# HarborC/PL-SLAM

Measured on NVIDIA H100. Metric: frames/sec (extract+match+pose-LM) 640x480, higher is better.
Workload: dtype u8/i32 front-end, f32 descriptors, f64 LM

## Files before the change

### include/plslam_b200.h

```cpp
#ifndef PLSLAM_B200_H
#define PLSLAM_B200_H
#include <stddef.h>
#include <stdint.h>
#ifdef __cplusplus
extern "C" {
#endif

#define PL_OK 0
#define PL_ERR_ARG (-1)
#define PL_ERR_CUDA (-2)
#define PL_ERR_CAPACITY (-3)

const char* pl_last_error(void);
int pl_version(void);
unsigned long long pl_launch_count(void);

typedef struct PLKeyPoint {
  float x, y, size, angle, response;
  int32_t octave, class_id;
} PLKeyPoint;

typedef struct PLOrbConfig {
  int width, height;
  int nfeatures;
// ... 61 lines not shown
                         const float* pt_inv_sigma2, const float* pt_Xw, int n_lines, const double* line_func,
                         const double* line_Xw, float* Tcw_out, uint8_t* pt_outlier, uint8_t* line_outlier,
                         int* iterations );
size_t pl_pose_optimization_scratch_doubles(int B, int cap_points, int cap_lines);
int pl_pose_optimization_dev(int mode, int B, const float* Tcw_in, const float* K, const int* n_points,
                             int cap_points, const float* pt_obs, const float* pt_inv_sigma2, const float* pt_Xw,
                             const int* n_lines, int cap_lines, const double* line_func, const double* line_Xw,
                             float* Tcw_out, uint8_t* pt_outlier, uint8_t* line_outlier, int* inliers,
                             int* iterations, double* scratch, void* stream);

typedef struct PLLineConfig {
  int width, height;
  int nfeatures;
  double min_line_length;
  int max_batch;
  int segment_cap;
  int lsd_used_in_global;
} PLLineConfig;
typedef struct PLLine PLLine;
int pl_line_create(const PLLineConfig* cfg, PLLine** out);
void pl_line_destroy(PLLine* h);
int pl_line_capacity(const PLLine* h);
int pl_line_extract(PLLine* h, const uint8_t* img, int stride, const uint8_t* mask, void* keylines, uint8_t* desc,
                    double* linefunc, int* n);
int pl_line_extract_batch(PLLine* h, const uint8_t* imgs, int stride, size_t frame_stride, int B, const uint8_t* mask,
                          void* keylines, uint8_t* desc, double* linefunc, int* n);
int pl_line_extract_batch_dev(PLLine* h, const uint8_t* imgs, int stride, size_t frame_stride, int B,
                              const uint8_t* mask, void* keylines, uint8_t* desc, double* linefunc, int* n, void* stream);
int pl_line_check_overflow(PLLine* h);
int pl_line_debug_segments(PLLine* h, int frame, float* out, int cap);
int pl_line_debug_scaled(PLLine* h, int frame, uint8_t* out, int* sw, int* sh);
int pl_line_debug_sobel(PLLine* h, int frame, short* dx, short* dy);
int pl_line_debug_order(PLLine* h, int frame, unsigned* out, int cap);
int pl_line_debug_ctl(PLLine* h, int frame, int* out, int nwords);

typedef struct PLFrontendConfig {
  int width, height, max_batch;
  int orb_nfeatures; float orb_scale_factor; int orb_nlevels, orb_ini_th, orb_min_th;
  int line_nfeatures; double line_min_length;
  int lm_cap_points, lm_cap_lines;
} PLFrontendConfig;
typedef struct PLFrontend PLFrontend;
int pl_frontend_create(const PLFrontendConfig* cfg, PLFrontend** out);
void pl_frontend_destroy(PLFrontend* h);
int pl_frontend_capacities(const PLFrontend* h, int* cap_keypoints, int* cap_lines);
int pl_frontend_set_pose_problems(PLFrontend* h, int B, const float* Tcw0, const float* K, const int* n_points,
                                  const float* pt_obs, const float* pt_inv_sigma2, const float* pt_Xw, const int* n_lines,
                                  const double* line_func, const double* line_Xw);
int pl_frontend_set_camera(PLFrontend* h, const float* K, const float* dist5);
long long pl_frontend_set_pose_problems_async(PLFrontend* h, int B, const float* Tcw0, const float* K, const int* n_points,
                                              const float* pt_obs, const float* pt_inv_sigma2, const float* pt_Xw,
                                              const int* n_lines, const double* line_func, const double* line_Xw, void* stream);
int pl_frontend_check_overflow(PLFrontend* h);
int pl_frontend_set_wrap(PLFrontend* h, int on);
int pl_frontend_set_tracking(PLFrontend* h, int on);
int pl_frontend_fetch_tracking(PLFrontend* h, int B, int which, int* point_match, int* n_point_matches, int* line_match,
                               int* n_line_matches, float* map_pos, uint8_t* point_in_view, uint8_t* line_in_view);
int pl_frontend_fetch_keys_un(PLFrontend* h, int B, PLKeyPoint* out);
int pl_frontend_run_dev(PLFrontend* h, const uint8_t* imgs, int stride, size_t frame_stride, int B, void* stream);
int pl_frontend_run(PLFrontend* h, const uint8_t* imgs, int stride, size_t frame_stride, int B, PLKeyPoint* kps,
                    uint8_t* desc, int* n, void* keylines, uint8_t* ldesc, double* linefunc, int* nl, int* pt_matches,
                    int* n_pt_matches, int* line_matches, int* n_line_matches, float* poses, int* inliers);
int pl_frontend_submit(PLFrontend* h, const uint8_t* imgs, int stride, size_t frame_stride, int B, PLKeyPoint* kps,
                       uint8_t* desc, int* n, void* keylines, uint8_t* ldesc, double* linefunc, int* nl, int* pt_matches,
                       int* n_pt_matches, int* line_matches, int* n_line_matches, float* poses, int* inliers);
int pl_frontend_wait(PLFrontend* h, int keep_in_flight);
// ... 216 lines not shown
```

### pl-slam_b200/binding.py

```python
import ctypes as C
import os
import numpy as np

_HERE = os.path.dirname(os.path.abspath(__file__))
LIB_PATH = os.environ.get("PLSLAM_B200_LIB") or os.path.join(_HERE, "libplslam_b200.so")

KP_DTYPE = np.dtype([("x", "<f4"), ("y", "<f4"), ("size", "<f4"), ("angle", "<f4"),
                     ("response", "<f4"), ("octave", "<i4"), ("class_id", "<i4")])


class PLError(RuntimeError):
    pass


class PLOrbConfig(C.Structure):
    _fields_ = [("width", C.c_int), ("height", C.c_int), ("nfeatures", C.c_int), ("scale_factor", C.c_float),
                ("nlevels", C.c_int), ("ini_th_fast", C.c_int), ("min_th_fast", C.c_int), ("max_batch", C.c_int),
                ("cell_slot_cap", C.c_int)]


_lib = None
vp = C.c_void_p


# ... 233 lines not shown


KEYLINE_DTYPE = np.dtype([("angle", "<f4"), ("class_id", "<i4"), ("octave", "<i4"), ("ptx", "<f4"), ("pty", "<f4"),
                          ("response", "<f4"), ("size", "<f4"), ("startPointX", "<f4"), ("startPointY", "<f4"),
                          ("endPointX", "<f4"), ("endPointY", "<f4"), ("sPointInOctaveX", "<f4"),
                          ("sPointInOctaveY", "<f4"), ("ePointInOctaveX", "<f4"), ("ePointInOctaveY", "<f4"),
                          ("lineLength", "<f4"), ("numOfPixels", "<i4")])


class PLLineConfig(C.Structure):
    _fields_ = [("width", C.c_int), ("height", C.c_int), ("nfeatures", C.c_int), ("min_line_length", C.c_double),
                ("max_batch", C.c_int), ("segment_cap", C.c_int), ("lsd_used_in_global", C.c_int)]


class LINEextractor:

    def __init__(self, numOctaves=1, scale=1.2, nLSDFeature=200, min_line_length=0.0, width=640, height=480, max_batch=1,
                 segment_cap=0):
        if numOctaves != 1 or int(scale) != 1:
            raise PLError("only numOctaves == 1 and int(scale) == 1 are supported (all reference configs)")
        self.cfg = PLLineConfig(width, height, nLSDFeature, float(min_line_length), max_batch, segment_cap, 0)
        self._h = vp()
        L = lib()
        L.pl_line_create.argtypes = [C.POINTER(PLLineConfig), C.POINTER(vp)]
        L.pl_line_destroy.argtypes = [vp]
        L.pl_line_capacity.argtypes = [vp]
        L.pl_line_extract.argtypes = [vp, vp, C.c_int, vp, vp, vp, vp, vp]
        L.pl_line_extract_batch.argtypes = [vp, vp, C.c_int, C.c_size_t, C.c_int, vp, vp, vp, vp, vp]
        L.pl_line_extract_batch_dev.argtypes = [vp, vp, C.c_int, C.c_size_t, C.c_int, vp, vp, vp, vp, vp, vp]
        L.pl_line_debug_segments.argtypes = [vp, C.c_int, vp, C.c_int]
        L.pl_line_debug_scaled.argtypes = [vp, C.c_int, vp, vp, vp]
        L.pl_line_debug_sobel.argtypes = [vp, C.c_int, vp, vp]
        L.pl_line_debug_order.argtypes = [vp, C.c_int, vp, C.c_int]
        check(L.pl_line_create(C.byref(self.cfg), C.byref(self._h)))
        self.capacity = check(L.pl_line_capacity(self._h))

    def __del__(self):
        if getattr(self, "_h", None) and self._h.value:
            lib().pl_line_destroy(self._h)
            self._h = vp()

    def __call__(self, image, mask=None):
        image = np.ascontiguousarray(image, np.uint8)
        if image.size == 0:
            return np.zeros(0, KEYLINE_DTYPE), np.zeros((0, 32), np.uint8), np.zeros((0, 3))
        if mask is not None and (mask.shape != image.shape or mask.dtype != np.uint8):
            raise PLError("Mask error while detecting lines: please check its dimensions and that data type is CV_8UC1")
        kl = np.zeros(self.capacity, KEYLINE_DTYPE); desc = np.zeros((self.capacity, 32), np.uint8)
        lf = np.zeros((self.capacity, 3), np.float64); n = C.c_int(0)
        m = None if mask is None else np.ascontiguousarray(mask)
        check(lib().pl_line_extract(self._h, _p(image), image.strides[0], _p(m), _p(kl), _p(desc), _p(lf), C.byref(n)))
        return kl[:n.value].copy(), desc[:n.value].copy(), lf[:n.value].copy()

    def extract_batch(self, images, mask=None):
        images = np.ascontiguousarray(images, np.uint8)
        B = images.shape[0]
        kl = np.zeros((B, self.capacity), KEYLINE_DTYPE); desc = np.zeros((B, self.capacity, 32), np.uint8)
        lf = np.zeros((B, self.capacity, 3), np.float64); n = np.zeros(B, np.int32)
        m = None if mask is None else np.ascontiguousarray(mask)
        check(lib().pl_line_extract_batch(self._h, _p(images), images.strides[1], images.strides[0], B, _p(m), _p(kl),
                                          _p(desc), _p(lf), _p(n)))
        return kl, desc, lf, n

    def extract_batch_dev(self, img_ptr, stride, frame_stride, B, mask_ptr, kl_ptr, desc_ptr, lf_ptr, n_ptr, stream=None):
        check(lib().pl_line_extract_batch_dev(self._h, img_ptr, stride, frame_stride, B, mask_ptr, kl_ptr, desc_ptr,
                                              lf_ptr, n_ptr, stream))

    def debug_segments(self, frame=0):
        n = check(lib().pl_line_debug_segments(self._h, frame, None, 0))
        out = np.zeros((max(n, 1), 4), np.float32)
        check(lib().pl_line_debug_segments(self._h, frame, _p(out), n))
        return out[:n]

    def debug_scaled(self, frame=0):
        sw, sh = C.c_int(), C.c_int()
        check(lib().pl_line_debug_scaled(self._h, frame, None, C.byref(sw), C.byref(sh)))
        out = np.zeros((sh.value, sw.value), np.uint8)
        check(lib().pl_line_debug_scaled(self._h, frame, _p(out), C.byref(sw), C.byref(sh)))
        return out

    def debug_sobel(self, frame=0):
        dx = np.zeros((self.cfg.height, self.cfg.width), np.int16); dy = np.zeros_like(dx)
        check(lib().pl_line_debug_sobel(self._h, frame, _p(dx), _p(dy)))
        return dx, dy

    def debug_order(self, frame=0):
        n = check(lib().pl_line_debug_order(self._h, frame, None, 0))
        out = np.zeros(max(n, 1), np.uint32)
        check(lib().pl_line_debug_order(self._h, frame, _p(out), n))
        return out[:n]


class PLFrontendConfig(C.Structure):
    _fields_ = [("width", C.c_int), ("height", C.c_int), ("max_batch", C.c_int), ("orb_nfeatures", C.c_int),
                ("orb_scale_factor", C.c_float), ("orb_nlevels", C.c_int), ("orb_ini_th", C.c_int), ("orb_min_th", C.c_int),
                ("line_nfeatures", C.c_int), ("line_min_length", C.c_double), ("lm_cap_points", C.c_int),
                ("lm_cap_lines", C.c_int)]


class Frontend:

    def __init__(self, width=640, height=480, max_batch=8, orb=(1000, 1.2, 8, 20, 7), lines=(200, 0.0), lm_caps=(512, 128)):
        self.cfg = PLFrontendConfig(width, height, max_batch, orb[0], orb[1], orb[2], orb[3], orb[4], lines[0], lines[1],
                                    lm_caps[0], lm_caps[1])
        self._h = vp()
        L = lib()
        L.pl_frontend_create.argtypes = [C.POINTER(PLFrontendConfig), C.POINTER(vp)]
        L.pl_frontend_destroy.argtypes = [vp]
        L.pl_frontend_capacities.argtypes = [vp, vp, vp]
        L.pl_frontend_set_pose_problems.argtypes = [vp, C.c_int] + [vp] * 9
        L.pl_frontend_run_dev.argtypes = [vp, vp, C.c_int, C.c_size_t, C.c_int, vp]
        L.pl_frontend_run.argtypes = [vp, vp, C.c_int, C.c_size_t, C.c_int] + [vp] * 13
        L.pl_frontend_io_bytes.argtypes = [vp, vp, vp]
        L.pl_frontend_fetch.argtypes = [vp, C.c_int] + [vp] * 12
        L.pl_frontend_set_timing.argtypes = [vp, C.c_int]
        L.pl_frontend_grow_ms.argtypes = [vp, vp]
        L.pl_frontend_grow_bytes_per_frame.argtypes = [vp]
        L.pl_frontend_grow_bytes_per_frame.restype = C.c_longlong
        L.pl_frontend_copy_poses_dev.argtypes = [vp, C.c_int, vp, vp]
        check(L.pl_frontend_create(C.byref(self.cfg), C.byref(self._h)))
        ck, cl = C.c_int(), C.c_int()
        check(L.pl_frontend_capacities(self._h, C.byref(ck), C.byref(cl)))
        self.capK, self.capL = ck.value, cl.value
# ... 924 lines not shown
```

### pl-slam_b200/csrc/common.cuh

```cuda
#pragma once
#include <cuda_runtime.h>
#include <stdint.h>
#include <stdio.h>
#include <string>
#include <atomic>
#include "../../include/plslam_b200.h"

namespace pl {

void set_error(const char* fmt, ...);
extern std::atomic<unsigned long long> g_launches;
inline void count_launch(int n = 1) { g_launches.fetch_add((unsigned long long)n, std::memory_order_relaxed); }

#define PL_CUDA(expr)                                                                       \
  do {                                                                                      \
    cudaError_t _e = (expr);                                                                \
    if (_e != cudaSuccess) {                                                                \
      pl::set_error("%s:%d %s -> %s", __FILE__, __LINE__, #expr, cudaGetErrorString(_e));   \
      return PL_ERR_CUDA;                                                                   \
    }                                                                                       \
  } while (0)

#define PL_LAUNCH_CHECK()                                                                   \
  do {                                                                                      \
    pl::count_launch();                                                                     \
    cudaError_t _e = cudaGetLastError();                                                    \
    if (_e != cudaSuccess) {                                                                \
      pl::set_error("%s:%d kernel launch -> %s", __FILE__, __LINE__, cudaGetErrorString(_e)); \
      return PL_ERR_CUDA;                                                                   \
    }                                                                                       \
  } while (0)

#define PL_ARG(cond)                                                                        \
  do {                                                                                      \
    if (!(cond)) {                                                                          \
      pl::set_error("%s:%d bad argument: %s", __FILE__, __LINE__, #cond);                   \
      return PL_ERR_ARG;                                                                    \
    }                                                                                       \
  } while (0)

int require_device();

template <typename T>
inline int dev_alloc(T** p, size_t n) {
  PL_CUDA(cudaMalloc((void**)p, n * sizeof(T)));
// ... 22 lines not shown
```

### pl-slam_b200/csrc/frontend.cu

```cuda

#include "common.cuh"
#include <vector>
#include <string>
#include <cstdio>
#include <string.h>

namespace pl {
__global__ void k_prev_matched_init(const PLKeyPoint* __restrict__ kps_prev, const int* __restrict__ n_prev, int cap, int B,
                                    float* __restrict__ pm) {
  const int b = blockIdx.y, i = blockIdx.x * blockDim.x + threadIdx.x;
  if (i < n_prev[b]) { pm[((long long)b * cap + i) * 2] = kps_prev[(long long)b * cap + i].x; pm[((long long)b * cap + i) * 2 + 1] = kps_prev[(long long)b * cap + i].y; }
}

__global__ void k_track_points(const PLKeyPoint* __restrict__ ku_prev, const PLKeyPoint* __restrict__ kraw_prev, const int* __restrict__ n_prev,
                               int cap, const float* __restrict__ Tcw0, const float* __restrict__ K, uint8_t* __restrict__ valid,
                               float* __restrict__ pos, int* __restrict__ oct, float* __restrict__ ang, float* __restrict__ proj,
                               float* __restrict__ vcos) {
  const int b = blockIdx.y, i = blockIdx.x * blockDim.x + threadIdx.x;
  if (i >= cap) return;
  const long long o = (long long)b * cap + i;
  const bool v = i < min(n_prev[b], cap);
  valid[o] = v ? 1 : 0;
  if (!v) return;
  const PLKeyPoint k = ku_prev[o];
// ... 103 lines not shown
  if (h->sLine) cudaStreamDestroy(h->sLine);
  if (h->sLm) cudaStreamDestroy(h->sLm);
  if (h->evStart) cudaEventDestroy(h->evStart);
  if (h->evLine) cudaEventDestroy(h->evLine);
  if (h->evLm) cudaEventDestroy(h->evLm);
  delete h;
}

extern "C" int pl_frontend_create(const PLFrontendConfig* cfg, PLFrontend** out) {
  PL_ARG(cfg && out && cfg->max_batch >= 1 && cfg->lm_cap_points >= 1 && cfg->lm_cap_lines >= 1);
  int rc = require_device();
  if (rc) return rc;
  PLFrontend* h = new PLFrontend;
  h->cfg = *cfg;
  h->B = cfg->max_batch;
#define FE_TRY(e) do { int _r = (e); if (_r) { pl_frontend_destroy(h); return _r; } } while (0)
#define FE_CUDA(e) do { cudaError_t _e = (e); if (_e != cudaSuccess) { set_error("%s -> %s", #e, cudaGetErrorString(_e)); pl_frontend_destroy(h); return PL_ERR_CUDA; } } while (0)
  PLOrbConfig oc = {cfg->width, cfg->height, cfg->orb_nfeatures, cfg->orb_scale_factor, cfg->orb_nlevels, cfg->orb_ini_th, cfg->orb_min_th, cfg->max_batch, 0};
  FE_TRY(pl_orb_create(&oc, &h->orb));
  PLLineConfig lc = {cfg->width, cfg->height, cfg->line_nfeatures, cfg->line_min_length, cfg->max_batch, 0, 0};
  FE_TRY(pl_line_create(&lc, &h->line));
  h->capK = pl_orb_capacity(h->orb); h->capL = pl_line_capacity(h->line);
  FE_CUDA(cudaStreamCreateWithFlags(&h->stream, cudaStreamNonBlocking));
  FE_CUDA(cudaStreamCreateWithFlags(&h->sLine, cudaStreamNonBlocking));
  FE_CUDA(cudaStreamCreateWithFlags(&h->sLm, cudaStreamNonBlocking));
  FE_CUDA(cudaEventCreateWithFlags(&h->evStart, cudaEventDisableTiming));
  FE_CUDA(cudaEventCreateWithFlags(&h->evLine, cudaEventDisableTiming));
  FE_CUDA(cudaEventCreateWithFlags(&h->evLm, cudaEventDisableTiming));
  { const char* e = getenv("PLSLAM_FRONTEND_OVERLAP"); h->overlap = !(e && e[0] == '0'); }
  {
    int dev = 0, sms = 132;
    FE_CUDA(cudaGetDevice(&dev));
    FE_CUDA(cudaDeviceGetAttribute(&sms, cudaDevAttrMultiProcessorCount, dev));
    h->serial_batch = 32 * sms;
  }
  if (const char* e = getenv("PLSLAM_FRONTEND_ORDER")) {
    const std::string o(e);
    if (o.size() == 3 && o.find('L') != std::string::npos && o.find('O') != std::string::npos && o.find('M') != std::string::npos) memcpy(h->order, o.data(), 3);
  }
  const size_t B = h->B, cK = h->capK, cL = h->capL, cp = cfg->lm_cap_points, cl = cfg->lm_cap_lines;
  FE_TRY(dev_alloc(&h->d_img, (size_t)cfg->width * cfg->height * B));
  FE_TRY(dev_alloc(&h->d_kps_prev, cK * (B + 1))); h->d_kps = h->d_kps_prev + cK;
  FE_TRY(dev_alloc(&h->d_desc_prev, cK * 32 * (B + 1))); h->d_desc = h->d_desc_prev + cK * 32;
  FE_TRY(dev_alloc(&h->d_n_prev, B + 1)); h->d_n = h->d_n_prev + 1;
  FE_CUDA(cudaMemset(h->d_n_prev, 0, sizeof(int) * (B + 1)));
  FE_TRY(dev_alloc(&h->d_ldesc_prev, cL * 32 * (B + 1))); h->d_ldesc = h->d_ldesc_prev + cL * 32;
  FE_TRY(dev_alloc(&h->d_nl_prev, B + 1)); h->d_nl = h->d_nl_prev + 1;
  FE_CUDA(cudaMemset(h->d_nl_prev, 0, sizeof(int) * (B + 1)));
  FE_TRY(dev_alloc(&h->d_kl_prev, cL * 68 * (B + 1))); h->d_kl = h->d_kl_prev + cL * 68;
  FE_TRY(dev_alloc(&h->d_lf, cL * 3 * B));
  FE_TRY(dev_alloc(&h->d_bounds, 4)); FE_TRY(dev_alloc(&h->d_pm, cK * 2 * B)); FE_TRY(dev_alloc(&h->d_m12, cK * B));
  FE_TRY(dev_alloc(&h->d_nm, B)); FE_TRY(dev_alloc(&h->d_scr, cK * 2 * B)); FE_TRY(dev_alloc(&h->d_lm, cL * B)); FE_TRY(dev_alloc(&h->d_nlm, B));
  float bounds[4] = {0.f, 0.f, (float)cfg->width, (float)cfg->height};
  FE_CUDA(cudaMemcpy(h->d_bounds, bounds, sizeof(bounds), cudaMemcpyHostToDevice));
  FE_TRY(dev_alloc(&h->d_T0, 16 * B)); FE_TRY(dev_alloc(&h->d_K, 4 * B)); FE_TRY(dev_alloc(&h->d_pobs, cp * 2 * B));
  FE_TRY(dev_alloc(&h->d_pw, cp * B)); FE_TRY(dev_alloc(&h->d_pX, cp * 3 * B)); FE_TRY(dev_alloc(&h->d_Tout, 16 * B * 2));
  FE_TRY(dev_alloc(&h->d_lfun, cl * 3 * B)); FE_TRY(dev_alloc(&h->d_lX, cl * 6 * B));
  FE_TRY(dev_alloc(&h->d_scratch, pl_pose_optimization_scratch_doubles((int)B, (int)cp, (int)cl)));
  FE_TRY(dev_alloc(&h->d_np, B)); FE_TRY(dev_alloc(&h->d_nl_lm, B)); FE_TRY(dev_alloc(&h->d_inl, B * 2)); FE_TRY(dev_alloc(&h->d_its, B * 2));
  FE_TRY(dev_alloc(&h->d_pout, cp * B * 2)); FE_TRY(dev_alloc(&h->d_lout, cl * B * 2));
  *out = h;
  return PL_OK;
}

extern "C" int pl_frontend_capacities(const PLFrontend* h, int* cap_keypoints, int* cap_lines) {
  PL_ARG(h);
  if (cap_keypoints) *cap_keypoints = h->capK;
// ... 434 lines not shown
```

### pl-slam_b200/csrc/line.cu

```cuda

#include "common.cuh"
#include "lsd_grow_core.cuh"
#include "libm_glibc.cuh"
#include <math.h>
#include <string.h>
#include <stdlib.h>
#include <vector>
#include <algorithm>

namespace pl {

constexpr double kPI = 3.14159265358979323846;
constexpr double kDegToRads = kPI / 180;
constexpr int kBins = 1024;
constexpr int kChunkRows = 8;


struct PLKeyLineRec {
  float angle; int class_id; int octave; float ptx, pty; float response; float size;
  float startPointX, startPointY, endPointX, endPointY;
  float sPointInOctaveX, sPointInOctaveY, ePointInOctaveX, ePointInOctaveY;
  float lineLength; int numOfPixels;
};
static_assert(sizeof(PLKeyLineRec) == 68, "KeyLine layout");

struct LineParams {
  int w, h, sw, sh, npx;
  int nchunk;
  int s_th;
  int min_reg_size;
  int seg_cap, capL, nfeatures;
  double min_line_length;
  double prec, prec_hi, p, density_th;
  float sure_ca2, sure_cn2;
};

__device__ __forceinline__ float fast_atan2_deg_l(float y, float x) {
  const float k = (float)(180.0 / 3.14159265358979323846);
  const float p1 = 0.9997878412794807f * k, p3 = -0.3258083974640975f * k;
  const float p5 = 0.1555786518463281f * k, p7 = -0.04432655554792128f * k;
  const float eps = 2.220446049250313e-16f;
  const float ax = fabsf(x), ay = fabsf(y);
  const float c = __fdiv_rn(fminf(ax, ay), __fadd_rn(fmaxf(ax, ay), eps)), c2 = __fmul_rn(c, c);
  float a = __fmul_rn(__fadd_rn(__fmul_rn(__fadd_rn(__fmul_rn(__fadd_rn(__fmul_rn(p7, c2), p5), c2), p3), c2), p1), c);
// ... 191 lines not shown
}

__global__ void __launch_bounds__(128) k_lsd_scatter(LineParams P, const int* __restrict__ S2, const int* __restrict__ maxs,
                                                     const int* __restrict__ offsets, unsigned* __restrict__ order) {
  __shared__ unsigned short cnt[4][kBins];
  const int wid = threadIdx.x >> 5, lane = threadIdx.x & 31;
  const int chunk = blockIdx.x * 4 + wid, f = blockIdx.y;
  for (int i = lane; i < kBins; i += 32) cnt[wid][i] = 0;
  __syncwarp();
  if (chunk >= P.nchunk) return;
  const int ms = maxs[f];
  const double max_grad = ms > 0 ? sqrt((double)ms / 4.0) : -1.0;
  const double bin_coef = (max_grad > 0) ? (double)(kBins - 1) / max_grad : 0.0;
  const int y0 = chunk * kChunkRows, y1 = min(y0 + kChunkRows, P.sh - 1);
  const int* SS = S2 + (long long)f * P.npx;
  const int* off = offsets + (long long)f * kBins * P.nchunk;
  unsigned* O = order + (long long)f * P.npx;
  const int n = (y1 - y0) * P.sw;
  const unsigned lt = (1u << lane) - 1u;
  for (int i0 = 0; i0 < n; i0 += 32) {
    int i = i0 + lane, bin = -1, pix = 0;
    if (i < n) {
      int y = y0 + i / P.sw, x = i % P.sw;
      pix = x | (y << 16);
      const int sv = SS[y * P.sw + x];
      if (sv > P.s_th) bin = s_bin(sv, bin_coef);
    }
    unsigned peers = __match_any_sync(0xffffffffu, bin);
    if (bin >= 0) O[off[bin * P.nchunk + chunk] + cnt[wid][bin] + __popc(peers & lt)] = (unsigned)pix;
    __syncwarp();
    if (bin >= 0 && (peers & lt) == 0) cnt[wid][bin] += (unsigned short)__popc(peers);
    __syncwarp();
  }
}

constexpr int kGrowQ = 256;
constexpr int kCommitBatches = 4;
constexpr unsigned kGrowWatchdog = 6u * 1000u * 1000u;
__device__ __forceinline__ int first_zero(unsigned m) { return m == 0xffffffffu ? 32 : __ffs(~m) - 1; }

__device__ __forceinline__ void warp_commit(const lg::Params& GP, const lg::Frame& Fm, float4* __restrict__ segs, int lane) {
  using namespace lg;
  const unsigned lt = (1u << lane) - 1u;
  for (int round = 0; round < kCommitBatches; round++) {
    const int F = ld_i(&Fm.ctl[C_FIN]);
    if (F >= Fm.n) return;
    const int i = F + lane;
    const unsigned w1 = (i < Fm.n) ? ld_u(&Fm.st[i]) : 0u;
    const unsigned s1 = w1 & ST_STATE;
    const int pre1 = first_zero(__ballot_sync(0xffffffffu, s1 == ST_NOOP || s1 == ST_EATEN || s1 == ST_DONE));
    if (pre1 == 0) return;
    __threadfence();
    unsigned w2 = 0u;
    bool ok = false;
    if (lane < pre1) { w2 = ld_u(&Fm.st[i]); ok = task_valid(GP, Fm, i, w2); }
    const int pre2 = min(pre1, first_zero(__ballot_sync(0xffffffffu, ok)));
    float4 sg;
    const bool has = (lane < pre2) && task_has_segment(Fm, w2, sg);
    const unsigned ms = __ballot_sync(0xffffffffu, has);
    const int ns = ld_i(&Fm.ctl[C_NS]);
    if (has) { const int slot = ns + __popc(ms & lt); if (slot < GP.seg_cap) segs[slot] = sg; }
    __syncwarp();
    if (lane == 0) {
      st_i(&Fm.ctl[C_NS], ns + __popc(ms));
      __threadfence();
      a_max(&Fm.ctl[C_FIN], F + pre2);
// ... 437 lines not shown
    s_norm2[0] = __fdiv_rn(1.f, sqrtf(temp));
  }
  __syncthreads();
  for (int i = tid; i < 72; i += 64) des[i] = __fmul_rn(des[i], s_norm2[0]);
  __syncthreads();
  if (tid < 32) {
    const float* f1 = &des[8 * c_comb[2 * tid]];
    const float* f2 = &des[8 * c_comb[2 * tid + 1]];
    unsigned r = 0;
#pragma unroll
    for (int i = 0; i < 8; i++) if (f1[i] > f2[i]) r += (1u << i);
    desc[((long long)f * P.capL + li) * 32 + tid] = (uint8_t)r;
  }
}

}

using namespace pl;

struct PLLine {
  PLLineConfig cfg;
  LineParams P;
  cudaStream_t stream = nullptr;
  uint8_t* d_scaled = nullptr;
  float2* d_seedcs = nullptr;
  lg::Params GP;
  int grow_warps_target = 132 * 16;
  int grow_wpf_max = 64;
  int grow_spec_max_batch = 0;
  size_t lane_warps = 0;
  int4* d_rec = nullptr; int* d_sq = nullptr;
  unsigned *d_st = nullptr, *d_pool = nullptr, *d_lanebuf = nullptr; int* d_ctl = nullptr; double* d_wtab = nullptr;
  GradRec* d_gtab = nullptr; float2* d_gtab_seed = nullptr;
  unsigned short* d_counts = nullptr;
  int *d_offsets = nullptr, *d_ndef = nullptr, *d_maxs = nullptr, *d_nseg = nullptr, *d_overflow = nullptr;
  unsigned* d_order = nullptr;
  float4* d_segs = nullptr;
  short2* d_dxy = nullptr;
  uint8_t* d_img = nullptr; PLKeyLineRec* d_kls = nullptr; uint8_t* d_desc = nullptr; double* d_lf = nullptr; int* d_nl = nullptr;
  uint8_t* d_mask = nullptr;
  size_t key_smem = 0;
  int last_B = 0;
  int timing = 0;
  cudaEvent_t ev0 = nullptr, ev1 = nullptr;
};

static const unsigned char h_comb[64] = {0, 1, 0, 2, 0, 3, 0, 4, 0, 5, 0, 6, 1, 2, 1, 3, 1, 4, 1, 5, 1, 6, 2, 3, 2, 4, 2, 5, 2, 6, 2, 7,
                                         2, 8, 3, 4, 3, 5, 3, 6, 3, 7, 3, 8, 4, 5, 4, 6, 4, 7, 4, 8, 5, 6, 5, 7, 5, 8, 6, 7, 6, 8, 7, 8};

extern "C" void pl_line_destroy(PLLine* h) {
  if (!h) return;
  cudaFree(h->d_gtab); cudaFree(h->d_gtab_seed); cudaFree(h->d_scaled); cudaFree(h->d_seedcs); cudaFree(h->d_rec); cudaFree(h->d_sq); cudaFree(h->d_st); cudaFree(h->d_pool); cudaFree(h->d_lanebuf); cudaFree(h->d_ctl); cudaFree(h->d_wtab); cudaFree(h->d_counts); cudaFree(h->d_offsets);
  cudaFree(h->d_ndef); cudaFree(h->d_maxs); cudaFree(h->d_nseg); cudaFree(h->d_overflow); cudaFree(h->d_order);
  cudaFree(h->d_segs); cudaFree(h->d_dxy); cudaFree(h->d_img); cudaFree(h->d_kls);
  cudaFree(h->d_desc); cudaFree(h->d_lf); cudaFree(h->d_nl); cudaFree(h->d_mask);
  if (h->stream) cudaStreamDestroy(h->stream);
  delete h;
}

extern "C" int pl_line_create(const PLLineConfig* cfg, PLLine** out) {
  PL_ARG(cfg && out);
  PL_ARG(cfg->width >= 64 && cfg->height >= 64 && cfg->width < 8000 && cfg->height < 8000 && cfg->nfeatures > 0 && cfg->max_batch >= 1);
  int rc = require_device();
  if (rc) return rc;
  PLLine* h = new PLLine;
  h->cfg = *cfg;
// ... 4 lines not shown
  P.nchunk = (P.sh - 1 + kChunkRows - 1) / kChunkRows;
  const double ANG_TH = 22.5, QUANT = 2.0;
  P.prec = kPI * ANG_TH / 180; P.p = ANG_TH / 180; P.density_th = 0.7;
  {
    const double twopi = 2 * kPI;
    double c = twopi - P.prec;
    while ((twopi - nextafter(c, 0.0)) <= P.prec) c = nextafter(c, 0.0);
    while (!((twopi - c) <= P.prec)) c = nextafter(c, 10.0);
    P.prec_hi = c;
  }
  {
    const double M = 0.05 * M_PI / 180.0, ca = cos(P.prec - M), cn = cos(P.prec + M);
    P.sure_ca2 = (float)(ca * ca); P.sure_cn2 = (float)(cn * cn);
  }
  const double rho = QUANT / sin(P.prec);
  int s = 0;
  while (sqrt((double)(s + 1) / 4.0) <= rho) s++;
  P.s_th = s;
  const double LOG_NT = 5 * (log10((double)P.sw) + log10((double)P.sh)) / 2 + log10(11.0);
  P.min_reg_size = (int)(size_t)(-LOG_NT / log10(P.p));
  P.seg_cap = cfg->segment_cap > 0 ? cfg->segment_cap : 8192;
  P.nfeatures = cfg->nfeatures; P.capL = cfg->nfeatures + 1; P.min_line_length = cfg->min_line_length;
  { size_t c2 = 1; while (c2 < (size_t)P.seg_cap) c2 <<= 1; h->key_smem = c2 * 8; }
  const size_t B = cfg->max_batch, npx = P.npx;
#define LN_TRY(e) do { int _r = (e); if (_r) { pl_line_destroy(h); return _r; } } while (0)
#define LN_CUDA(e) do { cudaError_t _e = (e); if (_e != cudaSuccess) { set_error("%s -> %s", #e, cudaGetErrorString(_e)); pl_line_destroy(h); return PL_ERR_CUDA; } } while (0)
  LN_CUDA(cudaStreamCreateWithFlags(&h->stream, cudaStreamNonBlocking));
  LN_TRY(dev_alloc(&h->d_scaled, npx * B)); LN_TRY(dev_alloc(&h->d_seedcs, npx * B)); LN_TRY(dev_alloc(&h->d_rec, npx * B));
  LN_TRY(dev_alloc(&h->d_sq, npx * B));
  {
    int dev = 0, sms = 132;
    cudaGetDevice(&dev); cudaDeviceGetAttribute(&sms, cudaDevAttrMultiProcessorCount, dev);
    h->grow_warps_target = sms * 16;
    if (const char* e = getenv("PLSLAM_LSD_GROW_WARPS")) { const int v = atoi(e); if (v > 0) h->grow_warps_target = v; }
    if (const char* e = getenv("PLSLAM_LSD_GROW_WPF")) { const int v = atoi(e); if (v > 0) h->grow_wpf_max = v; }
    if (const char* e = getenv("PLSLAM_LSD_GROW_SPEC_MAXB")) h->grow_spec_max_batch = atoi(e);
    lg::Params& G = h->GP;
    G.sw = P.sw; G.sh = P.sh; G.npx = P.npx; G.min_reg_size = P.min_reg_size; G.seg_cap = P.seg_cap;
    G.lane_cap = 1024; G.pool_cap = 4 * P.npx; G.window = 8192;
    if (const char* e = getenv("PLSLAM_LSD_GROW_WINDOW")) G.window = atoi(e);
    G.prec = P.prec; G.prec_hi = P.prec_hi; G.density_th = P.density_th;
    h->lane_warps = std::max<size_t>(std::min<size_t>(B * (size_t)h->grow_wpf_max, (size_t)h->grow_warps_target), B);
    LN_TRY(dev_alloc(&h->d_st, npx * B)); LN_TRY(dev_alloc(&h->d_pool, (size_t)G.pool_cap * B)); LN_TRY(dev_alloc(&h->d_ctl, (size_t)lg::kCtlStride * B));
    LN_TRY(dev_alloc(&h->d_lanebuf, h->lane_warps * 32 * (size_t)G.lane_cap));
    const int nw = 2 * kGradR * kGradR + 1;
    LN_TRY(dev_alloc(&h->d_wtab, (size_t)nw));
    k_lsd_wtab<<<(nw + 255) / 256, 256, 0, h->stream>>>(h->d_wtab, nw);
    LN_CUDA(cudaGetLastError());
    count_launch();
  }
  LN_TRY(dev_alloc(&h->d_counts, (size_t)kBins * P.nchunk * B)); LN_TRY(dev_alloc(&h->d_offsets, (size_t)kBins * P.nchunk * B));
  LN_TRY(dev_alloc(&h->d_ndef, B)); LN_TRY(dev_alloc(&h->d_maxs, B)); LN_TRY(dev_alloc(&h->d_nseg, B)); LN_TRY(dev_alloc(&h->d_overflow, 1));
  LN_TRY(dev_alloc(&h->d_order, npx * B)); LN_TRY(dev_alloc(&h->d_segs, (size_t)P.seg_cap * B));
  LN_TRY(dev_alloc(&h->d_dxy, (size_t)P.w * P.h * B));
  LN_CUDA(cudaMemset(h->d_overflow, 0, sizeof(int)));
  LN_TRY(dev_alloc(&h->d_gtab, (size_t)kGradN * kGradN)); LN_TRY(dev_alloc(&h->d_gtab_seed, (size_t)kGradN * kGradN));
  k_lsd_grad_table<<<(kGradN * kGradN + 255) / 256, 256, 0, h->stream>>>(h->d_gtab, h->d_gtab_seed);
  LN_CUDA(cudaGetLastError());
  LN_CUDA(cudaStreamSynchronize(h->stream));
  count_launch();
  {
    float gG[63], gL[21];
    double u = (7 * 3 - 1) / 2, sigma = (7 * 2 + 1) / 2, inv = -1 / (2 * sigma * sigma);
    for (int i = 0; i < 21; i++) { double d = i - u; gL[i] = (float)exp(d * d * inv); }
    u = (9 * 7 - 1) / 2; sigma = u; inv = -1 / (2 * sigma * sigma);
    for (int i = 0; i < 63; i++) { double d = i - u; gG[i] = (float)exp(d * d * inv); }
    LN_CUDA(cudaMemcpyToSymbol(c_gaussG, gG, sizeof(gG)));
    LN_CUDA(cudaMemcpyToSymbol(c_gaussL, gL, sizeof(gL)));
    LN_CUDA(cudaMemcpyToSymbol(c_comb, h_comb, sizeof(h_comb)));
  }
  LN_CUDA(cudaFuncSetAttribute(k_keylines, cudaFuncAttributeMaxDynamicSharedMemorySize, (int)h->key_smem));
  *out = h;
  return PL_OK;
}

extern "C" int pl_line_capacity(const PLLine* h) { return h ? h->P.capL : PL_ERR_ARG; }

extern "C" int pl_line_set_timing(PLLine* h, int on) {
  PL_ARG(h);
  if (on && !h->ev0) { PL_CUDA(cudaEventCreate(&h->ev0)); PL_CUDA(cudaEventCreate(&h->ev1)); }
  h->timing = on;
  return PL_OK;
}
extern "C" int pl_line_grow_ms(PLLine* h, float* ms) {
  PL_ARG(h && ms && h->ev0);
  PL_CUDA(cudaEventSynchronize(h->ev1));
  PL_CUDA(cudaEventElapsedTime(ms, h->ev0, h->ev1));
  return PL_OK;
}
extern "C" long long pl_line_grow_bytes_per_frame(const PLLine* h) { return h ? (long long)h->P.npx * 28 : 0; }

extern "C" int pl_line_extract_batch_dev(PLLine* h, const uint8_t* imgs, int stride, size_t frame_stride, int B,
                                         const uint8_t* mask, void* keylines, uint8_t* desc, double* linefunc, int* n,
                                         void* stream_) {
  PL_ARG(h && imgs && keylines && desc && linefunc && n && B >= 1 && B <= h->cfg.max_batch && stride >= h->cfg.width);
  cudaStream_t st = stream_ ? (cudaStream_t)stream_ : h->stream;
  const LineParams& P = h->P;
  h->last_B = B;
  PL_CUDA(cudaMemsetAsync(h->d_maxs, 0, sizeof(int) * B, st));
  k_lsd_scale<<<dim3((P.sw + 31) / 32, (P.sh + 31) / 32, B), 256, 0, st>>>(P, imgs, stride, (long long)frame_stride, h->d_scaled);
  PL_LAUNCH_CHECK();
  {
    const dim3 grd((P.sw + 255) / 256, (P.sh + 3) / 4, B);
    if (P.sw % 4 == 0)
      k_lsd_grad<true><<<grd, 256, 0, st>>>(P, h->d_scaled, reinterpret_cast<const float4*>(h->d_gtab), h->d_gtab_seed, h->d_rec, h->d_sq, h->d_seedcs, h->d_maxs);
    else
      k_lsd_grad<false><<<grd, 256, 0, st>>>(P, h->d_scaled, reinterpret_cast<const float4*>(h->d_gtab), h->d_gtab_seed, h->d_rec, h->d_sq, h->d_seedcs, h->d_maxs);
  }
  PL_LAUNCH_CHECK();
  k_lsd_hist<<<dim3(P.nchunk, B), 256, 0, st>>>(P, h->d_sq, h->d_maxs, h->d_counts);
  PL_LAUNCH_CHECK();
  k_lsd_scan<<<B, kBins, 0, st>>>(P, h->d_counts, h->d_offsets, h->d_ndef);
  PL_LAUNCH_CHECK();
  k_lsd_scatter<<<dim3((P.nchunk + 3) / 4, B), 128, 0, st>>>(P, h->d_sq, h->d_maxs, h->d_offsets, h->d_order);
  PL_LAUNCH_CHECK();
  if (B <= h->grow_spec_max_batch) {
    PL_CUDA(cudaMemsetAsync(h->d_st, 0, sizeof(unsigned) * (size_t)P.npx * B, st));
    k_lsd_grow_init<<<(B + 127) / 128, 128, 0, st>>>(h->d_ctl, B);
    PL_LAUNCH_CHECK();
    if (h->timing) PL_CUDA(cudaEventRecord(h->ev0, st));
    const int wpf = std::max(1, std::min(h->grow_wpf_max, h->grow_warps_target / B));
    k_lsd_grow<1><<<B * wpf, 32, 0, st>>>(P, h->GP, h->d_rec, h->d_seedcs, h->d_sq, h->d_order, h->d_ndef, h->d_st, h->d_pool, h->d_ctl,
                                          h->d_lanebuf, h->d_wtab, h->d_segs, h->d_nseg, h->d_overflow, B, wpf);
    PL_LAUNCH_CHECK();
  } else {
    if (h->timing) PL_CUDA(cudaEventRecord(h->ev0, st));
    static const int pre_maxb = getenv("PLSLAM_LSD_PRE_MAXB") ? atoi(getenv("PLSLAM_LSD_PRE_MAXB")) : 256;
    const int chunk = (int)std::min<long long>(B, 0xffffffffLL / P.npx);
    for (int b0 = 0; b0 < B; b0 += chunk) {
      const int nb = std::min(chunk, B - b0);
      const size_t po = (size_t)b0 * P.npx;
      if (B <= pre_maxb)
        k_lsd_grow_ordered<true><<<nb, 32, 0, st>>>(P, h->d_rec + po, h->d_sq + po, h->d_seedcs + po, h->d_order + po, h->d_ndef + b0,
                                                    h->d_pool + (size_t)b0 * h->GP.pool_cap, h->GP.pool_cap, h->d_st + po, h->d_wtab,
                                                    h->d_segs + (size_t)b0 * P.seg_cap, h->d_nseg + b0, h->d_overflow, nb);
      else
        k_lsd_grow_ordered<false><<<nb, 32, 0, st>>>(P, h->d_rec + po, h->d_sq + po, h->d_seedcs + po, h->d_order + po, h->d_ndef + b0,
                                                     h->d_pool + (size_t)b0 * h->GP.pool_cap, h->GP.pool_cap, h->d_st + po, h->d_wtab,
                                                     h->d_segs + (size_t)b0 * P.seg_cap, h->d_nseg + b0, h->d_overflow, nb);
    }
    PL_LAUNCH_CHECK();
  }
  if (h->timing) PL_CUDA(cudaEventRecord(h->ev1, st));
  k_keylines<<<B, 256, h->key_smem, st>>>(P, h->d_segs, h->d_nseg, mask, (PLKeyLineRec*)keylines, linefunc, n);
  PL_LAUNCH_CHECK();
  k_lbd_sobel<<<dim3((P.w + kSobOut - 1) / kSobOut, (P.h + kSobOut - 1) / kSobOut, B), 256, 0, st>>>(P, imgs, stride, (long long)frame_stride, h->d_dxy);
  PL_LAUNCH_CHECK();
  k_lbd_describe<<<dim3(P.capL, B), 64, 0, st>>>(P, (const PLKeyLineRec*)keylines, n, h->d_dxy, desc);
// ... 52 lines not shown
  return pl_line_extract_batch(h, img, stride, 0, 1, mask, keylines, desc, linefunc, n);
}

extern "C" int pl_line_debug_segments(PLLine* h, int frame, float* out, int cap) {
  PL_ARG(h && frame >= 0 && frame < h->last_B);
  int n = 0;
  PL_CUDA(cudaStreamSynchronize(h->stream));
  PL_CUDA(cudaMemcpy(&n, h->d_nseg + frame, sizeof(int), cudaMemcpyDeviceToHost));
  if (out && n) PL_CUDA(cudaMemcpy(out, h->d_segs + (size_t)frame * h->P.seg_cap, sizeof(float4) * std::min(n, cap), cudaMemcpyDeviceToHost));
  return n;
}
extern "C" int pl_line_debug_scaled(PLLine* h, int frame, uint8_t* out, int* sw, int* sh) {
  PL_ARG(h && frame >= 0 && frame < h->last_B && sw && sh);
  *sw = h->P.sw; *sh = h->P.sh;
  PL_CUDA(cudaStreamSynchronize(h->stream));
  if (out) PL_CUDA(cudaMemcpy(out, h->d_scaled + (size_t)frame * h->P.npx, h->P.npx, cudaMemcpyDeviceToHost));
  return PL_OK;
}
extern "C" int pl_line_debug_sobel(PLLine* h, int frame, short* dx, short* dy) {
  PL_ARG(h && frame >= 0 && frame < h->last_B && dx && dy);
  const size_t n = (size_t)h->P.w * h->P.h;
  PL_CUDA(cudaStreamSynchronize(h->stream));
  std::vector<short2> tmp(n);
  PL_CUDA(cudaMemcpy(tmp.data(), h->d_dxy + frame * n, n * sizeof(short2), cudaMemcpyDeviceToHost));
  for (size_t i = 0; i < n; i++) { dx[i] = tmp[i].x; dy[i] = tmp[i].y; }
  return PL_OK;
}
extern "C" int pl_line_debug_ctl(PLLine* h, int frame, int* out, int nwords) {
  PL_ARG(h && out && frame >= 0 && frame < h->cfg.max_batch && nwords > 0 && nwords <= lg::kCtlStride);
  PL_CUDA(cudaStreamSynchronize(h->stream));
  PL_CUDA(cudaMemcpy(out, h->d_ctl + (size_t)frame * lg::kCtlStride, sizeof(int) * nwords, cudaMemcpyDeviceToHost));
  return PL_OK;
}
extern "C" int pl_line_debug_order(PLLine* h, int frame, unsigned* out, int cap) {
  PL_ARG(h && frame >= 0 && frame < h->last_B);
  int n = 0;
  PL_CUDA(cudaStreamSynchronize(h->stream));
  PL_CUDA(cudaMemcpy(&n, h->d_ndef + frame, sizeof(int), cudaMemcpyDeviceToHost));
  if (out && n) {
    PL_CUDA(cudaMemcpy(out, h->d_order + (size_t)frame * h->P.npx, sizeof(unsigned) * std::min(n, cap), cudaMemcpyDeviceToHost));
    for (int i = 0; i < std::min(n, cap); i++) out[i] = (out[i] >> 16) * (unsigned)h->P.sw + (out[i] & 0xffffu);
  }
  return n;
}

#ifdef PL_GROW_STATS
extern "C" int pl_line_grow_stats(unsigned long long* out, int reset) {
  cudaDeviceSynchronize();
  if (out) cudaMemcpyFromSymbol(out, pl::ord::g_grow_stats, sizeof(unsigned long long) * 24);
  if (reset) { unsigned long long z[24] = {0}; cudaMemcpyToSymbol(pl::ord::g_grow_stats, z, sizeof(z)); }
  return 0;
}
#endif
```

Before: 10830.

## Fuse LSD seed histogram, scan and scatter into one thread-block-cluster kernel

Adds a kernel that uses an 8-CTA thread block cluster per frame to build the seed-gradient histogram, compute prefix offsets across the cluster through distributed shared memory, and scatter pixel coordinates into a shared-memory slice. The slice is then written to the global order array with vectorized stores. It replaces the three-launch hist/scan/scatter path, removing two launches and the global count and offset round trips. It is only chosen when the batch reaches 32 frames per SM, or when forced by an environment variable. The kernel needs a large dynamic shared-memory footprint, and debug entry points for the chosen path are added.

```diff
diff --git a/include/plslam_b200.h b/include/plslam_b200.h
--- a/include/plslam_b200.h
+++ b/include/plslam_b200.h
@@ -117,6 +117,8 @@
 int pl_line_debug_scaled(PLLine* h, int frame, uint8_t* out, int* sw, int* sh);
 int pl_line_debug_sobel(PLLine* h, int frame, short* dx, short* dy);
 int pl_line_debug_order(PLLine* h, int frame, unsigned* out, int cap);
+int pl_line_debug_seed_path(PLLine* h);
+int pl_line_debug_fill_order(PLLine* h, int byte);
 int pl_line_debug_ctl(PLLine* h, int frame, int* out, int nwords);
 
 typedef struct PLFrontendConfig {
diff --git a/pl-slam_b200/binding.py b/pl-slam_b200/binding.py
--- a/pl-slam_b200/binding.py
+++ b/pl-slam_b200/binding.py
@@ -289,6 +289,8 @@
         L.pl_line_debug_scaled.argtypes = [vp, C.c_int, vp, vp, vp]
         L.pl_line_debug_sobel.argtypes = [vp, C.c_int, vp, vp]
         L.pl_line_debug_order.argtypes = [vp, C.c_int, vp, C.c_int]
+        L.pl_line_debug_seed_path.argtypes = [vp]
+        L.pl_line_debug_fill_order.argtypes = [vp, C.c_int]
         check(L.pl_line_create(C.byref(self.cfg), C.byref(self._h)))
         self.capacity = check(L.pl_line_capacity(self._h))
 
@@ -346,6 +348,12 @@
         out = np.zeros(max(n, 1), np.uint32)
         check(lib().pl_line_debug_order(self._h, frame, _p(out), n))
         return out[:n]
+
+    def debug_seed_path(self):
+        return check(lib().pl_line_debug_seed_path(self._h))
+
+    def debug_fill_order(self, byte=0xFF):
+        check(lib().pl_line_debug_fill_order(self._h, byte))
 
 
 class PLFrontendConfig(C.Structure):
diff --git a/pl-slam_b200/csrc/common.cuh b/pl-slam_b200/csrc/common.cuh
--- a/pl-slam_b200/csrc/common.cuh
+++ b/pl-slam_b200/csrc/common.cuh
@@ -11,6 +11,7 @@
 void set_error(const char* fmt, ...);
 extern std::atomic<unsigned long long> g_launches;
 inline void count_launch(int n = 1) { g_launches.fetch_add((unsigned long long)n, std::memory_order_relaxed); }
+constexpr int kSerialFramesPerSM = 32;
 
 #define PL_CUDA(expr)                                                                       \
   do {                                                                                      \
diff --git a/pl-slam_b200/csrc/frontend.cu b/pl-slam_b200/csrc/frontend.cu
--- a/pl-slam_b200/csrc/frontend.cu
+++ b/pl-slam_b200/csrc/frontend.cu
@@ -159,7 +159,7 @@
     int dev = 0, sms = 132;
     FE_CUDA(cudaGetDevice(&dev));
     FE_CUDA(cudaDeviceGetAttribute(&sms, cudaDevAttrMultiProcessorCount, dev));
-    h->serial_batch = 32 * sms;
+    h->serial_batch = pl::kSerialFramesPerSM * sms;
   }
   if (const char* e = getenv("PLSLAM_FRONTEND_ORDER")) {
     const std::string o(e);
diff --git a/pl-slam_b200/csrc/line.cu b/pl-slam_b200/csrc/line.cu
--- a/pl-slam_b200/csrc/line.cu
+++ b/pl-slam_b200/csrc/line.cu
@@ -2,6 +2,7 @@
 #include "common.cuh"
 #include "lsd_grow_core.cuh"
 #include "libm_glibc.cuh"
+#include <cooperative_groups.h>
 #include <math.h>
 #include <string.h>
 #include <stdlib.h>
@@ -10,6 +11,7 @@
 
 namespace pl {
 
+namespace cg = cooperative_groups;
 constexpr double kPI = 3.14159265358979323846;
 constexpr double kDegToRads = kPI / 180;
 constexpr int kBins = 1024;
@@ -267,6 +269,117 @@
     if (bin >= 0 && (peers & lt) == 0) cnt[wid][bin] += (unsigned short)__popc(peers);
     __syncwarp();
   }
+}
+
+constexpr int kSeedCta = 8;
+constexpr int kSeedWarps = 32;
+__device__ __forceinline__ int seed_bin(int sv, int s_th, double bin_coef) { return sv > s_th ? s_bin(sv, bin_coef) : -1; }
+
+__global__ void __cluster_dims__(kSeedCta, 1, 1) __launch_bounds__(kSeedWarps * 32, 1)
+k_lsd_seed_order(LineParams P, int Q, int U, int S, const int* __restrict__ S2, const int* __restrict__ maxs,
+                 unsigned* __restrict__ order, int* __restrict__ ndef) {
+  extern __shared__ __align__(16) unsigned char seed_smem[];
+  unsigned* slice = reinterpret_cast<unsigned*>(seed_smem);
+  unsigned short* cnt = reinterpret_cast<unsigned short*>(slice + S);
+  int* tot = reinterpret_cast<int*>(cnt + kSeedWarps * kBins);
+  int* base = tot + kBins;
+  __shared__ int wsum[kSeedWarps];
+  __shared__ int s_nd;
+  cg::cluster_group cluster = cg::this_cluster();
+  const int r = (int)cluster.block_rank(), f = blockIdx.y;
+  const int tid = threadIdx.x, lane = tid & 31, wid = tid >> 5;
+  for (int i = tid; i < kSeedWarps * kBins / 2; i += kSeedWarps * 32) reinterpret_cast<unsigned*>(cnt)[i] = 0u;
+  const int ms = maxs[f];
+  const double max_grad = ms > 0 ? sqrt((double)ms / 4.0) : -1.0;
+  const double bin_coef = (max_grad > 0) ? (double)(kBins - 1) / max_grad : 0.0;
+  const int nrow = (P.sh - 1) * P.sw;
+  const int c1 = min((r + 1) * Q, nrow);
+  const int u0 = min(r * Q + wid * U, c1), u1 = min(u0 + U, c1);
+  const int* SS = S2 + (long long)f * P.npx;
+  __syncthreads();
+  unsigned* cw = reinterpret_cast<unsigned*>(cnt + wid * kBins);
+  for (int i0 = u0; i0 < u1; i0 += 128) {
+    int sv[4];
+#pragma unroll
+    for (int k = 0; k < 4; k++) { const int i = i0 + 32 * k + lane; sv[k] = i < u1 ? SS[i] : 0; }
+#pragma unroll
+    for (int k = 0; k < 4; k++) {
+      const int b = seed_bin(sv[k], P.s_th, bin_coef);
+      if (b >= 0) atomicAdd(&cw[b >> 1], 1u << ((b & 1) * 16));
+    }
+  }
+  __syncthreads();
+  const int bin = kBins - 1 - tid;
+  {
+    int run = 0;
+    for (int w = 0; w < kSeedWarps; w++) { unsigned short& c = cnt[w * kBins + bin]; const int v = c; c = (unsigned short)run; run += v; }
+    tot[bin] = run;
+  }
+  cluster.sync();
+  int pre = 0, all = 0;
+#pragma unroll
+  for (int q = 0; q < kSeedCta; q++) {
+    const int v = cluster.map_shared_rank(tot, q)[bin];
+    all += v;
+    if (q < r) pre += v;
+  }
+  int incl = all;
+#pragma unroll
+  for (int o = 1; o < 32; o <<= 1) { const int v = __shfl_up_sync(0xffffffffu, incl, o); if (lane >= o) incl += v; }
+  if (lane == 31) wsum[wid] = incl;
+  __syncthreads();
+  if (wid == 0) {
+    const int v = wsum[lane];
+    int in2 = v;
+#pragma unroll
+    for (int o = 1; o < 32; o <<= 1) { const int u = __shfl_up_sync(0xffffffffu, in2, o); if (lane >= o) in2 += u; }
+    wsum[lane] = in2 - v;
+    if (lane == 31) { s_nd = in2; if (r == 0) ndef[f] = in2; }
+  }
+  __syncthreads();
+  base[bin] = wsum[wid] + incl - all + pre;
+  __syncthreads();
+  unsigned short* wc = cnt + wid * kBins;
+  const unsigned lt = (1u << lane) - 1u;
+  int y = (u0 + lane) / P.sw, x = (u0 + lane) - y * P.sw;
+  for (int i0 = u0; i0 < u1; i0 += 128) {
+    int sv[4];
+#pragma unroll
+    for (int k = 0; k < 4; k++) { const int i = i0 + 32 * k + lane; sv[k] = i < u1 ? SS[i] : 0; }
+#pragma unroll
+    for (int k = 0; k < 4; k++) {
+      const int b = seed_bin(sv[k], P.s_th, bin_coef);
+      const unsigned peers = __match_any_sync(0xffffffffu, b);
+      if (b >= 0) {
+        const int pos = base[b] + wc[b] + __popc(peers & lt);
+        const int q = pos / S;
+        cluster.map_shared_rank(slice, q)[pos - q * S] = (unsigned)(x | (y << 16));
+      }
+      __syncwarp();
+      if (b >= 0 && (peers & lt) == 0) wc[b] += (unsigned short)__popc(peers);
+      __syncwarp();
+      x += 32;
+      if (x >= P.sw) { x -= P.sw; y++; }
+    }
+  }
+  cluster.sync();
+  const int n = min(S, s_nd - r * S);
+  if (n <= 0) return;
+  unsigned* g = order + (long long)f * P.npx + (long long)r * S;
+  const int head = min(n, (int)((4u - (unsigned)((reinterpret_cast<uintptr_t>(g) >> 2) & 3u)) & 3u));
+  if (tid < head) g[tid] = slice[tid];
+  const int nv = (n - head) >> 2;
+  uint4* g4 = reinterpret_cast<uint4*>(g + head);
+  if (head == 0) {
+    const uint4* s4 = reinterpret_cast<const uint4*>(slice);
+    for (int k = tid; k < nv; k += kSeedWarps * 32) g4[k] = s4[k];
+  } else {
+    for (int k = tid; k < nv; k += kSeedWarps * 32) {
+      const unsigned* s = slice + head + 4 * k;
+      g4[k] = make_uint4(s[0], s[1], s[2], s[3]);
+    }
+  }
+  for (int k = head + 4 * nv + tid; k < n; k += kSeedWarps * 32) g[k] = slice[k];
 }
 
 constexpr int kGrowQ = 256;
@@ -770,6 +883,10 @@
   int4* d_rec = nullptr; int* d_sq = nullptr;
   unsigned *d_st = nullptr, *d_pool = nullptr, *d_lanebuf = nullptr; int* d_ctl = nullptr; double* d_wtab = nullptr;
   GradRec* d_gtab = nullptr; float2* d_gtab_seed = nullptr;
+  int seed_q = 0, seed_u = 0, seed_s = 0, seed_clusters = 0;
+  int seed_min_batch = 132 * kSerialFramesPerSM;
+  int last_seed_cluster = 0;
+  size_t seed_smem = 0;
   unsigned short* d_counts = nullptr;
   int *d_offsets = nullptr, *d_ndef = nullptr, *d_maxs = nullptr, *d_nseg = nullptr, *d_overflow = nullptr;
   unsigned* d_order = nullptr;
@@ -840,6 +957,7 @@
     int dev = 0, sms = 132;
     cudaGetDevice(&dev); cudaDeviceGetAttribute(&sms, cudaDevAttrMultiProcessorCount, dev);
     h->grow_warps_target = sms * 16;
+    h->seed_min_batch = sms * kSerialFramesPerSM;
     if (const char* e = getenv("PLSLAM_LSD_GROW_WARPS")) { const int v = atoi(e); if (v > 0) h->grow_warps_target = v; }
     if (const char* e = getenv("PLSLAM_LSD_GROW_WPF")) { const int v = atoi(e); if (v > 0) h->grow_wpf_max = v; }
     if (const char* e = getenv("PLSLAM_LSD_GROW_SPEC_MAXB")) h->grow_spec_max_batch = atoi(e);
@@ -878,6 +996,22 @@
     LN_CUDA(cudaMemcpyToSymbol(c_comb, h_comb, sizeof(h_comb)));
   }
   LN_CUDA(cudaFuncSetAttribute(k_keylines, cudaFuncAttributeMaxDynamicSharedMemorySize, (int)h->key_smem));
+  {
+    const int nrow = (P.sh - 1) * P.sw, maxdef = (P.sw - 1) * (P.sh - 1);
+    h->seed_q = (nrow + kSeedCta - 1) / kSeedCta;
+    h->seed_u = ((h->seed_q + kSeedWarps - 1) / kSeedWarps + 31) & ~31;
+    h->seed_s = ((maxdef + kSeedCta - 1) / kSeedCta + 3) & ~3;
+    h->seed_smem = (size_t)h->seed_s * sizeof(unsigned) + (size_t)kSeedWarps * kBins * sizeof(unsigned short) + 2 * kBins * sizeof(int);
+    int dev = 0, smem_max = 0;
+    cudaGetDevice(&dev);
+    cudaDeviceGetAttribute(&smem_max, cudaDevAttrMaxSharedMemoryPerBlockOptin, dev);
+    if (h->seed_q <= 65535 && h->seed_smem + 2 * 1024 <= (size_t)smem_max) {
+      LN_CUDA(cudaFuncSetAttribute(k_lsd_seed_order, cudaFuncAttributeMaxDynamicSharedMemorySize, (int)h->seed_smem));
+      cudaLaunchConfig_t lc = {};
+      lc.gridDim = dim3(kSeedCta, 1, 1); lc.blockDim = dim3(kSeedWarps * 32, 1, 1); lc.dynamicSmemBytes = h->seed_smem;
+      LN_CUDA(cudaOccupancyMaxActiveClusters(&h->seed_clusters, (void*)k_lsd_seed_order, &lc));
+    }
+  }
   *out = h;
   return PL_OK;
 }
@@ -902,9 +1036,18 @@
                                          const uint8_t* mask, void* keylines, uint8_t* desc, double* linefunc, int* n,
                                          void* stream_) {
   PL_ARG(h && imgs && keylines && desc && linefunc && n && B >= 1 && B <= h->cfg.max_batch && stride >= h->cfg.width);
+  const char* so = getenv("PLSLAM_LSD_SEED_ORDER");
+  const bool force_cluster = so && strcmp(so, "cluster") == 0, force_legacy = so && strcmp(so, "legacy") == 0;
+  if (force_cluster && h->seed_clusters == 0) {
+    set_error("PLSLAM_LSD_SEED_ORDER=cluster: a %dx%d scaled frame does not fit k_lsd_seed_order (%zu B of shared memory, %d pixels per CTA)",
+              h->P.sw, h->P.sh, h->seed_smem, h->seed_q);
+    return PL_ERR_ARG;
+  }
+  const bool cluster = h->seed_clusters > 0 && !force_legacy && (force_cluster || B >= h->seed_min_batch);
   cudaStream_t st = stream_ ? (cudaStream_t)stream_ : h->stream;
   const LineParams& P = h->P;
   h->last_B = B;
+  h->last_seed_cluster = cluster;
   PL_CUDA(cudaMemsetAsync(h->d_maxs, 0, sizeof(int) * B, st));
   k_lsd_scale<<<dim3((P.sw + 31) / 32, (P.sh + 31) / 32, B), 256, 0, st>>>(P, imgs, stride, (long long)frame_stride, h->d_scaled);
   PL_LAUNCH_CHECK();
@@ -916,12 +1059,18 @@
       k_lsd_grad<false><<<grd, 256, 0, st>>>(P, h->d_scaled, reinterpret_cast<const float4*>(h->d_gtab), h->d_gtab_seed, h->d_rec, h->d_sq, h->d_seedcs, h->d_maxs);
   }
   PL_LAUNCH_CHECK();
-  k_lsd_hist<<<dim3(P.nchunk, B), 256, 0, st>>>(P, h->d_sq, h->d_maxs, h->d_counts);
-  PL_LAUNCH_CHECK();
-  k_lsd_scan<<<B, kBins, 0, st>>>(P, h->d_counts, h->d_offsets, h->d_ndef);
-  PL_LAUNCH_CHECK();
-  k_lsd_scatter<<<dim3((P.nchunk + 3) / 4, B), 128, 0, st>>>(P, h->d_sq, h->d_maxs, h->d_offsets, h->d_order);
-  PL_LAUNCH_CHECK();
+  if (cluster) {
+    k_lsd_seed_order<<<dim3(kSeedCta, B), kSeedWarps * 32, h->seed_smem, st>>>(P, h->seed_q, h->seed_u, h->seed_s, h->d_sq, h->d_maxs,
+                                                                             h->d_order, h->d_ndef);
+    PL_LAUNCH_CHECK();
+  } else {
+    k_lsd_hist<<<dim3(P.nchunk, B), 256, 0, st>>>(P, h->d_sq, h->d_maxs, h->d_counts);
+    PL_LAUNCH_CHECK();
+    k_lsd_scan<<<B, kBins, 0, st>>>(P, h->d_counts, h->d_offsets, h->d_ndef);
+    PL_LAUNCH_CHECK();
+    k_lsd_scatter<<<dim3((P.nchunk + 3) / 4, B), 128, 0, st>>>(P, h->d_sq, h->d_maxs, h->d_offsets, h->d_order);
+    PL_LAUNCH_CHECK();
+  }
   if (B <= h->grow_spec_max_batch) {
     PL_CUDA(cudaMemsetAsync(h->d_st, 0, sizeof(unsigned) * (size_t)P.npx * B, st));
     k_lsd_grow_init<<<(B + 127) / 128, 128, 0, st>>>(h->d_ctl, B);
@@ -1040,11 +1189,24 @@
   PL_CUDA(cudaMemcpy(out, h->d_ctl + (size_t)frame * lg::kCtlStride, sizeof(int) * nwords, cudaMemcpyDeviceToHost));
   return PL_OK;
 }
+extern "C" int pl_line_debug_seed_path(PLLine* h) {
+  PL_ARG(h);
+  return h->last_seed_cluster;
+}
+extern "C" int pl_line_debug_fill_order(PLLine* h, int byte) {
+  PL_ARG(h);
+  PL_CUDA(cudaStreamSynchronize(h->stream));
+  PL_CUDA(cudaMemset(h->d_order, byte, sizeof(unsigned) * (size_t)h->P.npx * h->cfg.max_batch));
+  PL_CUDA(cudaMemset(h->d_ndef, byte, sizeof(int) * (size_t)h->cfg.max_batch));
+  PL_CUDA(cudaDeviceSynchronize());
+  return PL_OK;
+}
 extern "C" int pl_line_debug_order(PLLine* h, int frame, unsigned* out, int cap) {
   PL_ARG(h && frame >= 0 && frame < h->last_B);
   int n = 0;
   PL_CUDA(cudaStreamSynchronize(h->stream));
   PL_CUDA(cudaMemcpy(&n, h->d_ndef + frame, sizeof(int), cudaMemcpyDeviceToHost));
+  if (n < 0) { set_error("seed order of frame %d: ndef = %d was not written by the last call", frame, n); return PL_ERR_ARG; }
   if (out && n) {
     PL_CUDA(cudaMemcpy(out, h->d_order + (size_t)frame * h->P.npx, sizeof(unsigned) * std::min(n, cap), cudaMemcpyDeviceToHost));
     for (int i = 0; i < std::min(n, cap); i++) out[i] = (out[i] >> 16) * (unsigned)h->P.sw + (out[i] & 0xffffu);
```

Measured after the change: 11810, median of 6. 1.09x the previous value.
